# KlrShaK/opencv-SimpleSLAM

Measured on AMD Instinct MI355X. Metric: frames/sec ALIKED+LightGlue @1241x376, higher is better.
Workload: dtype f32 (contractions: f16 hi/lo split operands, f32 accumulate; 3 MFMA per product, 2 in attention's P.V = precision 'f16x3p1', the default since r05: profiles/r05_flip_soak.md, r06_flip_soak.md); 1 GPU; C2/C4: synthetic 1241x376x3 uint8 frame stream, ALIKED-n16 extract + LightGlue match (t-1,t), 2048 kpts/frame, min_conf 0.7, random-init weights; inputs resident in HBM before the timed region, features and matches left on the device (the `pcie` leg times the same pipeline with per-round H2D of the frames and D2H of {count, pairs}); max_kpts=2048, lightglue_layers_executed=9, pairs_per_lightglue_launch=8, frames_per_aliked_launch=8

## Files before the change

### opencv-simpleslam_amd/csrc/al_plan.hpp

```cpp
#pragma once
#include <algorithm>
#include <cstddef>
#include <cstdio>

namespace sslam {

constexpr int AL_LONG_SIDE = 1024;
constexpr int AL_PAD_DIV = 32;
constexpr int MAX_FRAMES = 16;
constexpr int B1_SW = 30;
constexpr int B2_SW = 30;
constexpr int DCN3_CS = 1;
constexpr int DCN4_CS = 4;
constexpr int AGG_PRE = 13;
constexpr int ST_W = 32, ST_H = 8;
constexpr int PRE_LDS_MAX = 48 * 1024;
constexpr int NHALO = 10;
constexpr int NW_R = 48, NW_OW = 64 - 2 * NHALO, NW_OH = NW_R - 2 * NHALO;
constexpr int HBINS = 4096;
constexpr int COLLECT_PPT = 16;
constexpr int SEL_CAP = 8192;
constexpr int EDGE_CAP = 2048;
constexpr int CAND_CAP = 1024 * 1024;
constexpr int REFINE_KPB = 32;
constexpr int SDDH_KSPLIT = 4;

constexpr int al_cdiv(int a, int b) { return (a + b - 1) / b; }

struct Dims {
// ... 14 lines not shown
    int b1_strips, b1_nblk, b1_hs, b1_nb;
    int b2_strips, b2_nblk, b2_hs, b2_nb, b2_waves, b2_gx;
    int H2, W2, HW2, H3, W3, HW3, H4, W4, HW4;
    int pool3_gx, pool4_gx;
    int off3_gx, dcn3_gx, off4_gx, dcn4_gx;
    float mo3, mo4, mo;
    int gate2_gx, gate3_gx, gate4_gx, gate34_gx;
    float sy2, sx2, sy8, sx8, sy32, sx32;
    int agg_pre_gx;
    int tail_gx, tail_gy;
    int nbx, nby, n_tiles, nms_gx;
    int npx, collect_gx;
    ALAggTile agg_tile;
    float scale_x, scale_y;
    int pre_tw, pre_th, pre_gx, pre_gy, pre_cols, pre_rows, pre_raw, pre_lds;
};

inline ALPlan al_plan(int H, int W, int C, int F) {
    ALPlan p{};
    p.F = F; p.KF = SDDH_KSPLIT * F;
    Dims& d = p.d;
    d.H = H; d.W = W; d.C = C;
    const double ar = (double)W / (double)H;
    if (ar > 1.0) { d.h = (int)(AL_LONG_SIDE / ar); d.w = AL_LONG_SIDE; }
    else { d.h = AL_LONG_SIDE; d.w = (int)(AL_LONG_SIDE * ar); }
    const double fy = (double)H / d.h, fx = (double)W / d.w;
    p.blur = (fy > fx ? fy : fx) > 1.0;
    const double sgy = (fy - 1.0) / 2.0 > 0.001 ? (fy - 1.0) / 2.0 : 0.001, sgx = (fx - 1.0) / 2.0 > 0.001 ? (fx - 1.0) / 2.0 : 0.001;
    p.sy = (float)sgy; p.sx = (float)sgx;
    const double ksy = 2.0 * 2 * sgy, ksx = 2.0 * 2 * sgx;
// ... 18 lines not shown
    p.b2_waves = p.b2_strips * p.b2_nb * F;
    p.b2_gx = al_cdiv(p.b2_waves, 4);
    p.H3 = Hp / 8; p.W3 = Wp / 8; p.HW3 = p.H3 * p.W3;
    p.H4 = Hp / 32; p.W4 = Wp / 32; p.HW4 = p.H4 * p.W4;
    p.pool3_gx = al_cdiv(32 * p.HW3, 256); p.pool4_gx = al_cdiv(64 * p.HW4, 256);
    p.off3_gx = al_cdiv(p.W3, 32); p.dcn3_gx = DCN3_CS * al_cdiv(p.W3, 32);
    p.off4_gx = al_cdiv(p.W4, 32); p.dcn4_gx = DCN4_CS * al_cdiv(p.W4, 32);
    p.mo3 = (float)(p.H3 > p.W3 ? p.H3 : p.W3) / 4.0f;
    p.mo4 = (float)(p.H4 > p.W4 ? p.H4 : p.W4) / 4.0f;
    p.gate2_gx = al_cdiv(p.HW2, 256); p.gate3_gx = al_cdiv(32 * p.HW3, 256); p.gate4_gx = al_cdiv(32 * p.HW4, 256);
    p.gate34_gx = p.gate3_gx + p.gate4_gx;
    auto step = [](int full, int S) { return (float)(full / S - 1) / (float)(full - 1); };
    p.sy2 = step(Hp, 2); p.sx2 = step(Wp, 2); p.sy8 = step(Hp, 8); p.sx8 = step(Wp, 8);
    p.sy32 = step(Hp, 32); p.sx32 = step(Wp, 32);
    p.agg_pre_gx = al_cdiv(p.HW2 + p.HW3 + p.HW4, 256);
    p.tail_gx = al_cdiv(Wp, ST_W); p.tail_gy = al_cdiv(Hp, ST_H);
    p.nbx = al_cdiv(d.w, NW_OW); p.nby = al_cdiv(d.h, NW_OH); p.n_tiles = p.nbx * p.nby;
    p.nms_gx = al_cdiv(p.n_tiles, 4);
    p.npx = d.h * d.w;
    p.collect_gx = al_cdiv(p.npx, 256 * COLLECT_PPT);
    p.mo = (float)(d.h > d.w ? d.h : d.w) / 4.0f;
    p.agg_tile = F >= 4 ? ALAggTile::T64x128 : ALAggTile::T64x64;
    p.scale_x = (float)d.w / (float)W; p.scale_y = (float)d.h / (float)H;
    {
        static constexpr int ladder[][2] = {{64, 8}, {32, 8}, {32, 4}, {16, 4}, {16, 2}, {8, 2}, {8, 1}, {4, 1}};
        const int rx = p.blur ? p.kx / 2 : 0, ry = p.blur ? p.ky / 2 : 0, planes = C == 1 ? 1 : 3;
        for (const auto& t : ladder) {
            p.pre_tw = t[0]; p.pre_th = t[1];
            p.pre_cols = (int)(fx * (t[0] - 1)) + 4;
            p.pre_rows = (int)(fy * (t[1] - 1)) + 4 + 2 * ry;
// ... 84 lines not shown
```

### opencv-simpleslam_amd/csrc/aliked_kernels.hip

```cpp
#include "common.hpp"
#include "al_plan.hpp"
#include "gemm_f32.hpp"
#include <type_traits>
#include "gemm_f16x3.hpp"

namespace {

using sslam::f32x16;
using sslam::acc_row;
using sslam::GemmSmem;
using sslam::GemmA;
using sslam::gemm_mainloop;
using sslam::Dims;
using sslam::MAX_FRAMES; using sslam::B1_SW; using sslam::B2_SW; using sslam::DCN3_CS; using sslam::DCN4_CS; using sslam::AGG_PRE;
using sslam::ST_W; using sslam::ST_H; using sslam::NHALO; using sslam::NW_R; using sslam::NW_OW; using sslam::NW_OH; using sslam::HBINS;
using sslam::COLLECT_PPT; using sslam::SEL_CAP; using sslam::EDGE_CAP; using sslam::REFINE_KPB; using sslam::SDDH_KSPLIT;

constexpr float SELU_SCALE = 1.0507009873554804934193349852946f;
constexpr float SELU_ALPHA = 1.6732632423543772848170429916717f;
__device__ __forceinline__ float selu(float x) {
    return SELU_SCALE * (x > 0.0f ? x : SELU_ALPHA * (__expf(x) - 1.0f));
}

__device__ __forceinline__ float selu_precise(float x) {
// ... 772 lines not shown
        for (int j = 0; j < MT * 4; ++j) {
            const int qi = wave * MT * 4 + j, m = qi / 16, r = qi % 16, co = 32 * (mt0 + m) + acc_row(r, lane);
            const int o = (m * 16 + r) * 64 + lane;
            float v = ((red[o] + red[o + MT * 1024]) + red[o + 2 * MT * 1024]) + red[o + 3 * MT * 1024];
            v += beta[co];
            if (RC) v += bd[co];
            v = selu(v);
            out[(size_t)co * HW + pix] = v;
            if (out_cl) out_cl[(size_t)pix * COUT + co] = v;
        }
    }
}



template <int CIN>
__global__ __launch_bounds__(256) void al_gate_kernel(const float* __restrict__ in, float* __restrict__ out,
                                                      int HW, const float* __restrict__ w ,
                                                      float* __restrict__ out_cl , size_t fs) {
    __shared__ float cl[256 * 33];
    const int p0 = blockIdx.x * blockDim.x, p = p0 + threadIdx.x, pc = min(p, HW - 1);
    in = fsh(in, blockIdx.y, fs); out = fsh(out, blockIdx.y, fs); out_cl = fsh(out_cl, blockIdx.y, fs);
    float v[CIN];
#pragma unroll
    for (int ci = 0; ci < CIN; ++ci) v[ci] = in[(size_t)ci * HW + pc];
    float acc[32];
#pragma unroll
    for (int o = 0; o < 32; ++o) acc[o] = 0.0f;
#pragma unroll
    for (int ci = 0; ci < CIN; ++ci) {
        const float* wp = w + ci * 32;
#pragma unroll
        for (int o = 0; o < 32; ++o) acc[o] = fmaf(v[ci], wp[o], acc[o]);
    }
#pragma unroll
    for (int o = 0; o < 32; ++o) { acc[o] = selu(acc[o]); cl[threadIdx.x * 33 + o] = acc[o]; }
    if (p < HW) {
#pragma unroll
        for (int o = 0; o < 32; ++o) out[(size_t)o * HW + p] = acc[o];
    }
    __syncthreads();
    const int npx = min(256, HW - p0);
    float* dst = out_cl + (size_t)p0 * 32;
    for (int i = threadIdx.x; i < npx * 8; i += 256) {
        const int q = i >> 3, c4 = (i & 7) * 4;
        *reinterpret_cast<float4*>(dst + (size_t)q * 32 + c4) = make_float4(cl[q * 33 + c4], cl[q * 33 + c4 + 1], cl[q * 33 + c4 + 2], cl[q * 33 + c4 + 3]);
    }
}

struct GateSmall { const float* in; float* out; int CIN; int HW; const float* w; float* out_cl; };
__global__ void al_gate_small_kernel(GateSmall a, GateSmall b, int blocks_a, size_t fs) {
    const bool second = (int)blockIdx.x >= blocks_a;
    const GateSmall& q = second ? b : a;
    const int i = ((int)blockIdx.x - (second ? blocks_a : 0)) * blockDim.x + threadIdx.x;
    const int CIN = q.CIN, HW = q.HW;
    if (i >= 32 * HW) return;
    const float* __restrict__ in = fsh(q.in, blockIdx.y, fs);
    float* __restrict__ out = fsh(q.out, blockIdx.y, fs);
    float* __restrict__ out_cl = fsh0(q.out_cl, blockIdx.y, fs);
    const float* __restrict__ w = q.w;
    const int co = i / HW, p = i % HW;
    float a0 = 0.0f, a1 = 0.0f;
#pragma unroll 8
    for (int ci = 0; ci < CIN; ci += 2) {
        a0 = fmaf(in[(size_t)ci * HW + p], w[ci * 32 + co], a0);
        a1 = fmaf(in[(size_t)(ci + 1) * HW + p], w[(ci + 1) * 32 + co], a1);
    }
    const float v = selu(a0 + a1);
    out[i] = v;
    out_cl[(size_t)p * 32 + co] = v;
}

struct Pyr {
    const float* x1; const float* g2; const float* g3; const float* g4;
    const float* w1;
    int Hp, Wp;
    float* g1cl;
    float sy2, sx2, sy8, sx8, sy32, sx32;
    const float *g2cl, *g3cl, *g4cl;
    const float *pre2, *pre3, *pre4;
};

__device__ __forceinline__ Pyr pyr_at(Pyr P, int f, size_t fs) {
    P.x1 = fsh(P.x1, f, fs); P.g2 = fsh(P.g2, f, fs); P.g3 = fsh(P.g3, f, fs); P.g4 = fsh(P.g4, f, fs);
    P.g1cl = fsh(P.g1cl, f, fs); P.g2cl = fsh(P.g2cl, f, fs); P.g3cl = fsh(P.g3cl, f, fs); P.g4cl = fsh(P.g4cl, f, fs);
    P.pre2 = fsh(P.pre2, f, fs); P.pre3 = fsh(P.pre3, f, fs); P.pre4 = fsh(P.pre4, f, fs);
    return P;
}

struct UpTap { int o00, o01, o10, o11; float w00, w01, w10, w11; };

__device__ __forceinline__ UpTap up_tap(int y, int x, int Hp, int Wp, int S, float sy, float sx) {
    const int ih = Hp / S, iw = Wp / S;
    const float fy = sy * (float)y, fx = sx * (float)x;
    const int y0 = (int)fy, x0 = (int)fx;
    const int y1 = y0 + (y0 < ih - 1), x1 = x0 + (x0 < iw - 1);
    const float ly = fy - (float)y0, lx = fx - (float)x0, hy = 1.0f - ly, hx = 1.0f - lx;
    UpTap t;
    t.o00 = y0 * iw + x0; t.o01 = y0 * iw + x1; t.o10 = y1 * iw + x0; t.o11 = y1 * iw + x1;
    t.w00 = hx; t.w01 = lx; t.w10 = hy; t.w11 = ly;
    return t;
}
__device__ __forceinline__ float up_eval_cl(const float* __restrict__ p, const UpTap& t, int c) {
    return t.w10 * (t.w00 * p[t.o00 * 32 + c] + t.w01 * p[t.o01 * 32 + c]) +
           t.w11 * (t.w00 * p[t.o10 * 32 + c] + t.w01 * p[t.o11 * 32 + c]);
}
__device__ __forceinline__ float up_eval(const float* __restrict__ p, const UpTap& t) {
    return t.w10 * (t.w00 * p[t.o00] + t.w01 * p[t.o01]) + t.w11 * (t.w00 * p[t.o10] + t.w01 * p[t.o11]);
}

constexpr int PRE_UNROLL = 32;
__global__ __launch_bounds__(256) void al_agg_pre_kernel(const float* __restrict__ g2cl , const float* __restrict__ g3cl,
                                                         const float* __restrict__ g4cl, const float* __restrict__ ws0 ,
                                                         float* __restrict__ pre2, float* __restrict__ pre3, float* __restrict__ pre4,
                                                         int Hp, int Wp, size_t fs) {
    const int f = blockIdx.y;
    const int n2 = (Hp / 2) * (Wp / 2), n3 = (Hp / 8) * (Wp / 8), n4 = (Hp / 32) * (Wp / 32);
    int i = blockIdx.x * blockDim.x + threadIdx.x;
    const float* g; float* pre; int S, lvl;
    if (i < n2) { g = g2cl; pre = pre2; S = 2; lvl = 1; }
    else if (i < n2 + n3) { i -= n2; g = g3cl; pre = pre3; S = 8; lvl = 2; }
    else if (i < n2 + n3 + n4) { i -= n2 + n3; g = g4cl; pre = pre4; S = 32; lvl = 3; }
    else return;
    g = fsh(g, f, fs); pre = fsh(pre, f, fs);
    const int ih = Hp / S, iw = Wp / S, n = ih * iw;
    const int y = i / iw, x = i % iw;
    const int xr = x + (x < iw - 1), yd = y + (y < ih - 1);
    const int ia = y * iw + x, ib = y * iw + xr, ic = yd * iw + x, id = yd * iw + xr;
    float pr[8] = {}, ss = 0.0f, hh = 0.0f, vv = 0.0f, d1 = 0.0f, d2 = 0.0f;
    const float* w = ws0 + lvl * 32 * 8;
#pragma unroll PRE_UNROLL
    for (int c = 0; c < 32; ++c) {
        const float* gc = g + (size_t)c * n;
        const float av = gc[ia], bv = gc[ib], cv = gc[ic], dv = gc[id];
        ss = fmaf(av, av, ss); hh = fmaf(av, bv, hh); vv = fmaf(av, cv, vv);
        d1 = fmaf(av, dv, d1); d2 = fmaf(bv, cv, d2);
#pragma unroll
        for (int o = 0; o < 8; ++o) pr[o] = fmaf(av, w[c * 8 + o], pr[o]);
    }
#pragma unroll
    for (int o = 0; o < 8; ++o) pre[(size_t)o * n + i] = pr[o];
    pre[(size_t)8 * n + i] = ss; pre[(size_t)9 * n + i] = hh; pre[(size_t)10 * n + i] = vv;
    pre[(size_t)11 * n + i] = d1; pre[(size_t)12 * n + i] = d2;
}

__device__ __forceinline__ void agg_level(const float* __restrict__ pre, int n, const UpTap& t, float (&s)[8], float& n2) {
#pragma unroll
    for (int o = 0; o < 8; ++o) s[o] += up_eval(pre + (size_t)o * n, t);
    const float w00 = t.w10 * t.w00, w01 = t.w10 * t.w01, w10 = t.w11 * t.w00, w11 = t.w11 * t.w01;
    const float* S = pre + (size_t)8 * n; const float* H = pre + (size_t)9 * n; const float* V = pre + (size_t)10 * n;
    const float* D1 = pre + (size_t)11 * n; const float* D2 = pre + (size_t)12 * n;
    const float sq = (w00 * w00 * S[t.o00] + w01 * w01 * S[t.o01]) + (w10 * w10 * S[t.o10] + w11 * w11 * S[t.o11]);
    const float cr = ((w00 * w01) * H[t.o00] + (w10 * w11) * H[t.o10]) + ((w00 * w10) * V[t.o00] + (w01 * w11) * V[t.o01]) +
                     ((w00 * w11) * D1[t.o00] + (w01 * w10) * D2[t.o00]);
    n2 += fmaf(2.0f, cr, sq);
}

constexpr int AGG1_UNROLL = 2;
// ... 5 lines not shown
    __shared__ float g1s[256 * 33];
    const int x = blockIdx.x * blockDim.x + threadIdx.x, y = blockIdx.y;
    const bool live = x < P.Wp;
    const size_t HW = (size_t)P.Hp * P.Wp, pix = (size_t)y * P.Wp + min(x, P.Wp - 1);
    float xv[16];
#pragma unroll
    for (int k = 0; k < 16; ++k) xv[k] = P.x1[k * HW + pix];
    float s[8];
#pragma unroll
    for (int o = 0; o < 8; ++o) s[o] = 0.0f;
    float n2 = 0.0f;
#pragma unroll AGG1_UNROLL
    for (int c = 0; c < 32; ++c) {
        float a = 0.0f;
#pragma unroll
        for (int k = 0; k < 16; ++k) a = fmaf(xv[k], P.w1[k * 32 + c], a);
        a = selu_precise(a);
        g1s[threadIdx.x * 33 + c] = a;
        n2 = fmaf(a, a, n2);
#pragma unroll
        for (int o = 0; o < 8; ++o) s[o] = fmaf(a, ws0[c * 8 + o], s[o]);
    }
    const UpTap t2 = up_tap(y, x, P.Hp, P.Wp, 2, P.sy2, P.sx2), t3 = up_tap(y, x, P.Hp, P.Wp, 8, P.sy8, P.sx8),
                t4 = up_tap(y, x, P.Hp, P.Wp, 32, P.sy32, P.sx32);
    agg_level(P.pre2, (int)(HW / 4), t2, s, n2);
    agg_level(P.pre3, (int)(HW / 64), t3, s, n2);
    agg_level(P.pre4, (int)(HW / 1024), t4, s, n2);
    if (live) {
#pragma unroll
        for (int o = 0; o < 8; ++o) s8[o * HW + pix] = selu_precise(s[o]);
        rnorm[pix] = 1.0f / fmaxf(sqrtf(n2), 1e-12f);
    }
    __builtin_amdgcn_fence(__ATOMIC_RELEASE, "workgroup");
    __builtin_amdgcn_s_barrier();
    __builtin_amdgcn_fence(__ATOMIC_ACQUIRE, "workgroup");
    typedef float f32x4_t __attribute__((ext_vector_type(4)));
    const int npx = min(256, P.Wp - (int)(blockIdx.x * blockDim.x));
    float* dst = P.g1cl + ((size_t)y * P.Wp + blockIdx.x * blockDim.x) * 32;
    for (int i = threadIdx.x; i < npx * 8; i += 256) {
        const int p = i >> 3, c4 = (i & 7) * 4;
        const f32x4_t v = {g1s[p * 33 + c4], g1s[p * 33 + c4 + 1], g1s[p * 33 + c4 + 2], g1s[p * 33 + c4 + 3]};
        *reinterpret_cast<f32x4_t*>(dst + (size_t)p * 32 + c4) = v;
    }
}

__device__ __forceinline__ float2 feat_pair(const Pyr& P, const float* __restrict__ rnorm, int pl, int pt,
                                            int y, int x, int lane) {
    const int yp = y + pt, xp = x + pl;
    const size_t pix = (size_t)yp * P.Wp + xp;
    float a, b;
    const int c = lane & 31;
    if (lane < 32) {
        a = P.g1cl[pix * 32 + c];
        b = up_eval_cl(P.g3cl, up_tap(yp, xp, P.Hp, P.Wp, 8, P.sy8, P.sx8), c);
    } else {
        a = up_eval_cl(P.g2cl, up_tap(yp, xp, P.Hp, P.Wp, 2, P.sy2, P.sx2), c);
        b = up_eval_cl(P.g4cl, up_tap(yp, xp, P.Hp, P.Wp, 32, P.sy32, P.sx32), c);
// ... 757 lines not shown
struct sslam_aliked {
    sslam_ctx* ctx = nullptr;
    int max_h = 0, max_w = 0, max_kpts = 0;
    int max_frames = 1;
    size_t fs = 0;
    int Hp_cap = 0, Wp_cap = 0;
    sslam::OwnedSlab slab;
    float* blob = nullptr;
    ALConvW b1c1, b1c2, b2c1, b2c2;
    const float *b2dw, *b2db;
    ALDcnW b3c1, b3c2, b4c1, b4c2;
    const float *b3dw, *b3db, *b4dw, *b4db;
    _Float16 *b3c1of, *b3c2of, *b4c1of, *b4c2of;
    _Float16 *b3c1f, *b3c2f, *b4c1f, *b4c2f;
    const float *gw1, *gw2, *gw3, *gw4;
    const float *sh0, *sh2, *sh4, *sh6;
    const float *d_ow, *d_ob, *d_w2, *d_b2, *d_sf, *d_agg;
    ALCtrl* ctrl;
    uint8_t* in_u8;
    float *img, *x1, *x2, *p3, *off, *t3, *x3, *p4, *t4, *x4, *g2, *g3, *g4;
    float *s8, *rnorm, *score, *nms, *bsum, *gk, *g1cl, *g2cl, *g3cl, *g4cl, *pre2, *pre3, *pre4;
    unsigned long long* cand;
    unsigned* hist;
    int cand_cap;
    int* kp_index;
    int* range_sticky;
    unsigned long long* sel_keys;
    float *kp_norm, *kp_score, *patch, *h32, *pos, *sampled, *feats, *raw;
    _Float16 *d_sf_s, *d_agg_s;
    _Float16* b2c2f;
// ... 39 lines not shown
    (void)hipGetLastError();
    const Dims& d = p.d;
    const sslam::ALKptPlan& k = g->kp;
    const int F = p.F, KF = p.KF, NK = k.NK;
    const size_t fs = g->fs;
    const dim3 b256(256);
    hipLaunchKernelGGL(al_reset_kernel, dim3(F), b256, 0, s, g->ctrl, g->hist, fs, g->gk, p.kx, p.sx, p.ky, p.sy);

    hipLaunchKernelGGL(al_preprocess_kernel, dim3(p.pre_gx, p.pre_gy, F), b256, (size_t)p.pre_lds, s, srcs, g->img, d, g->gk, p.kx, p.ky,
                       p.blur, PreTile{p.pre_tw, p.pre_th, p.pre_cols, p.pre_rows, p.pre_raw}, fs);
    hipLaunchKernelGGL(al_block1_rows_kernel, dim3(p.b1_strips, p.b1_nb, F), dim3(64), 0, s, g->img, g->x1, d.Hp, d.Wp, p.b1_hs,
                       g->b1c1.w, g->b1c1.a, g->b1c1.b, g->b1c2f, g->b1c2.a, g->b1c2.b, g->ctrl, fs);
    hipLaunchKernelGGL(al_block2_rows_kernel, dim3(p.b2_gx), b256, B2_LDS, s, g->x1, g->x2, p.H2, p.W2, p.b2_hs, p.b2_nb, p.b2_strips,
                       p.b2_waves, g->b2c1f, g->b2c2f, g->b2c1.a, g->b2c1.b, g->b2db, g->b2c2.a, g->b2c2.b, g->ctrl, fs);
    const dim3 off3 = dim3(p.off3_gx, p.H3, F), dcn3 = dim3(p.dcn3_gx, p.H3, F);
    hipLaunchKernelGGL(al_avgpool_kernel, dim3(p.pool3_gx, F), b256, 0, s, g->x2, g->p3, 32, p.H2, p.W2, 4, fs, g->p3cl);
    hipLaunchKernelGGL((al_offset_conv_h_kernel<32>), off3, b256, 0, s, g->p3cl, g->off, p.H3, p.W3, g->b3c1of, g->b3c1.ob, p.mo3, g->ctrl, fs);
    hipLaunchKernelGGL((al_dcn_h_kernel<32, 64, 0, DCN3_CS>), dcn3, b256, 0, s, g->p3cl, g->off, nullptr, p.H3, p.W3, g->b3c1f, g->b3c1.b, nullptr, g->t3, g->t3cl, g->ctrl, fs);
    hipLaunchKernelGGL((al_offset_conv_h_kernel<64>), off3, b256, 0, s, g->t3cl, g->off, p.H3, p.W3, g->b3c2of, g->b3c2.ob, p.mo3, g->ctrl, fs);
    hipLaunchKernelGGL((al_dcn_h_kernel<64, 64, 32, DCN3_CS>), dcn3, b256, 0, s, g->t3cl, g->off, g->p3cl, p.H3, p.W3, g->b3c2f, g->b3c2.b, g->b3db, g->x3, nullptr, g->ctrl, fs);
    const dim3 off4 = dim3(p.off4_gx, p.H4, F), dcn4 = dim3(p.dcn4_gx, p.H4, F);
    sslam::graph_cut(s);
    hipLaunchKernelGGL(al_avgpool_kernel, dim3(p.pool4_gx, F), b256, 0, s, g->x3, g->p4, 64, p.H3, p.W3, 4, fs, g->p4cl);
    hipLaunchKernelGGL((al_offset_conv_h_kernel<64>), off4, b256, 0, s, g->p4cl, g->off, p.H4, p.W4, g->b4c1of, g->b4c1.ob, p.mo4, g->ctrl, fs);
    hipLaunchKernelGGL((al_dcn_h_kernel<64, 128, 0, DCN4_CS>), dcn4, b256, 0, s, g->p4cl, g->off, nullptr, p.H4, p.W4, g->b4c1f, g->b4c1.b, nullptr, g->t4, g->t4cl, g->ctrl, fs);
    hipLaunchKernelGGL((al_offset_conv_h_kernel<128>), off4, b256, 0, s, g->t4cl, g->off, p.H4, p.W4, g->b4c2of, g->b4c2.ob, p.mo4, g->ctrl, fs);
    hipLaunchKernelGGL((al_dcn_h_kernel<128, 128, 64, DCN4_CS>), dcn4, b256, 0, s, g->t4cl, g->off, g->p4cl, p.H4, p.W4, g->b4c2f, g->b4c2.b, g->b4db, g->x4, nullptr, g->ctrl, fs);
    hipLaunchKernelGGL(al_gate_kernel<32>, dim3(p.gate2_gx, F), b256, 0, s, g->x2, g->g2, p.HW2, g->gw2, g->g2cl, fs);
    hipLaunchKernelGGL(al_gate_small_kernel, dim3(p.gate34_gx, F), b256, 0, s, GateSmall{g->x3, g->g3, 64, p.HW3, g->gw3, g->g3cl},
                       GateSmall{g->x4, g->g4, 128, p.HW4, g->gw4, g->g4cl}, p.gate3_gx, fs);
    Pyr P{g->x1, g->g2, g->g3, g->g4, g->gw1, d.Hp, d.Wp, g->g1cl};
    P.sy2 = p.sy2; P.sx2 = p.sx2; P.sy8 = p.sy8; P.sx8 = p.sx8; P.sy32 = p.sy32; P.sx32 = p.sx32;
    P.g2cl = g->g2cl; P.g3cl = g->g3cl; P.g4cl = g->g4cl;
    P.pre2 = g->pre2; P.pre3 = g->pre3; P.pre4 = g->pre4;
    hipLaunchKernelGGL(al_agg_pre_kernel, dim3(p.agg_pre_gx, F), b256, 0, s, g->g2, g->g3, g->g4, g->sh0, g->pre2, g->pre3, g->pre4,
                       d.Hp, d.Wp, fs);
    hipLaunchKernelGGL(al_aggregate_kernel, dim3(p.pad_gx, d.Hp, F), b256, 0, s, P, g->sh0, g->s8, g->rnorm, fs);
    hipLaunchKernelGGL(al_score_tail_kernel, dim3(p.tail_gx, p.tail_gy, F), dim3(ST_T), 0, s, g->s8, d.Hp, d.Wp, g->sh2, g->sh4, g->sh6,
                       g->score, d.h, d.w, d.pl, d.pt, fs);
    hipLaunchKernelGGL(al_nms_wave_kernel, dim3(p.nms_gx, F), b256, 0, s, g->score, d.h, d.w, p.nbx, p.n_tiles, g->nms, g->bsum, 0.2f,
                       g->cand, g->cand_cap, g->ctrl, g->hist, fs);
    sslam::graph_cut(s);
    hipLaunchKernelGGL(al_collect_kernel, dim3(p.collect_gx, F), b256, 0, s, g->nms, p.npx, 0.0f, 1, g->bsum, p.n_tiles, g->cand,
                       g->cand_cap, g->ctrl, g->hist, fs);
    hipLaunchKernelGGL(al_select_kernel, dim3(F), dim3(1024), SEL_LDS, s, g->cand, g->cand_cap, n_limit, g->sel_keys, g->ctrl, g->hist, fs);
    hipLaunchKernelGGL(al_refine_kernel, dim3(k.refine_gx, F), b256, 0, s, g->score, d.h, d.w, g->sel_keys, g->kp_index, g->kp_norm,
                       g->kp_score, g->ctrl, fs);
    hipLaunchKernelGGL(al_patch_kernel, dim3(k.patch_gx, F), b256, 0, s, P, g->rnorm, d.pl, d.pt, d.h, d.w, g->kp_norm, g->patch, g->ctrl, fs);
    hipLaunchKernelGGL((al_gemm_kernel<64, 64, 1, 1>), dim3(1, k.rows64, KF), b256, 0, s, g->patch, 1152, g->d_ow, nullptr, 32, g->h32,
                       1, NK, 0, g->ctrl, SDDH_KSPLIT, fs);
    hipLaunchKernelGGL(al_offsets_kernel, dim3(k.offsets_gx, F), b256, 0, s, g->h32, NK, g->d_ob, g->d_w2, g->d_b2, g->kp_norm, d.h, d.w,
// ... 48 lines not shown
    g->ctx = ctx; g->max_h = max_h; g->max_w = max_w; g->max_kpts = max_kpts; g->max_frames = max_frames;
    g->kp = sslam::al_kpt_plan(max_kpts);
    g->Hp_cap = sslam::AL_LONG_SIDE + sslam::AL_PAD_DIV; g->Wp_cap = sslam::AL_LONG_SIDE + sslam::AL_PAD_DIV;
    const sslam::ALExtents e = sslam::al_extents((size_t)g->Hp_cap * g->Wp_cap, (size_t)max_h * max_w, (size_t)max_kpts);
    g->cand_cap = sslam::CAND_CAP;
    auto bind_shared = [&](sslam::Slab& A) {
        g->blob = A.take<float>(n_floats);
        g->d_sf_s = A.take<_Float16>(2 * 128 * 128); g->d_agg_s = A.take<_Float16>((size_t)2 * 128 * 2048);
        g->b2c2f = A.take<_Float16>(2 * 32 * 288);
        g->b1c2f = A.take<_Float16>(5 * 2 * 64 * 8);
        g->b2c1f = A.take<_Float16>(10 * 2 * 64 * 8);
        g->b3c1f = A.take<_Float16>((size_t)(9 * 2 + 0) * 2 * 2 * 512); g->b3c2f = A.take<_Float16>((size_t)(9 * 4 + 2) * 2 * 2 * 512);
        g->b4c1f = A.take<_Float16>((size_t)(9 * 4 + 0) * 4 * 2 * 512); g->b4c2f = A.take<_Float16>((size_t)(9 * 8 + 4) * 4 * 2 * 512);
        g->b3c1of = A.take<_Float16>(18 * 2 * 512); g->b3c2of = A.take<_Float16>(36 * 2 * 512); g->b4c1of = A.take<_Float16>(36 * 2 * 512); g->b4c2of = A.take<_Float16>(72 * 2 * 512);
        g->gk = A.take<float>(64);
        g->range_sticky = A.take<int>(4);
    };
    auto bind_frame = [&](sslam::Slab& A) {
        g->ctrl = A.take<ALCtrl>(e.ctrl);
        g->in_u8 = A.take<uint8_t>(e.in_u8);
        g->img = A.take<float>(e.img);
        g->x1 = A.take<float>(e.x1); g->x2 = A.take<float>(e.x2);
        g->p3 = A.take<float>(e.p3); g->off = A.take<float>(e.off);
        g->t3 = A.take<float>(e.t3); g->x3 = A.take<float>(e.x3);
        g->p3cl = A.take<float>(e.p3cl); g->t3cl = A.take<float>(e.t3cl);
        g->p4cl = A.take<float>(e.p4cl); g->t4cl = A.take<float>(e.t4cl);
        g->p4 = A.take<float>(e.p4); g->t4 = A.take<float>(e.t4); g->x4 = A.take<float>(e.x4);
        g->g2 = A.take<float>(e.g2); g->g3 = A.take<float>(e.g3); g->g4 = A.take<float>(e.g4);
        g->g2cl = A.take<float>(e.g2cl); g->g3cl = A.take<float>(e.g3cl); g->g4cl = A.take<float>(e.g4cl);
        g->s8 = A.take<float>(e.s8); g->rnorm = A.take<float>(e.rnorm); g->g1cl = A.take<float>(e.g1cl);
// ... 26 lines not shown
        hipStream_t s = ctx->stream;
        SSLAM_HIP_CHECK(hipMemsetAsync(g->range_sticky, 0, 4 * sizeof(int), s));
        hipLaunchKernelGGL(al_conv32_wfrag_kernel, dim3(sslam::cdiv(32 * 288, 256)), dim3(256), 0, s, g->b2c2.w, g->b2c2f, g->range_sticky);
        hipLaunchKernelGGL(al_conv16_wfrag_kernel, dim3(sslam::cdiv(5 * 64 * 8, 256)), dim3(256), 0, s, g->b1c2.w, g->b1c2f, g->range_sticky);
        hipLaunchKernelGGL(al_conv32p_wfrag_kernel, dim3(sslam::cdiv(10 * 64 * 8, 256)), dim3(256), 0, s, g->b2c1.w, g->b2dw, g->b2c1f, g->range_sticky);
        hipLaunchKernelGGL(al_split_kernel, dim3(sslam::cdiv(128 * 128, 256)), dim3(256), 0, s, g->d_sf, g->d_sf_s, (size_t)128 * 128, g->range_sticky);
        hipLaunchKernelGGL(al_split_kernel, dim3(sslam::cdiv(128 * 2048, 256)), dim3(256), 0, s, g->d_agg, g->d_agg_s, (size_t)128 * 2048, g->range_sticky);
        hipLaunchKernelGGL((al_dcn_wfrag_kernel<32, 64, 0>), dim3(sslam::cdiv((9 * 2 + 0) * 2 * 512, 256)), dim3(256), 0, s, g->b3c1.w, g->b3c1.a, nullptr, g->b3c1f, g->range_sticky);
        hipLaunchKernelGGL((al_dcn_wfrag_kernel<64, 64, 32>), dim3(sslam::cdiv((9 * 4 + 2) * 2 * 512, 256)), dim3(256), 0, s, g->b3c2.w, g->b3c2.a, g->b3dw, g->b3c2f, g->range_sticky);
        hipLaunchKernelGGL((al_dcn_wfrag_kernel<64, 128, 0>), dim3(sslam::cdiv((9 * 4 + 0) * 4 * 512, 256)), dim3(256), 0, s, g->b4c1.w, g->b4c1.a, nullptr, g->b4c1f, g->range_sticky);
        hipLaunchKernelGGL((al_dcn_wfrag_kernel<128, 128, 64>), dim3(sslam::cdiv((9 * 8 + 4) * 4 * 512, 256)), dim3(256), 0, s, g->b4c2.w, g->b4c2.a, g->b4dw, g->b4c2f, g->range_sticky);
        hipLaunchKernelGGL(al_offc_wfrag_kernel<32>, dim3(sslam::cdiv(18 * 512, 256)), dim3(256), 0, s, g->b3c1.ow, g->b3c1of, g->range_sticky);
        hipLaunchKernelGGL(al_offc_wfrag_kernel<64>, dim3(sslam::cdiv(36 * 512, 256)), dim3(256), 0, s, g->b3c2.ow, g->b3c2of, g->range_sticky);
        hipLaunchKernelGGL(al_offc_wfrag_kernel<64>, dim3(sslam::cdiv(36 * 512, 256)), dim3(256), 0, s, g->b4c1.ow, g->b4c1of, g->range_sticky);
        hipLaunchKernelGGL(al_offc_wfrag_kernel<128>, dim3(sslam::cdiv(72 * 512, 256)), dim3(256), 0, s, g->b4c2.ow, g->b4c2of, g->range_sticky);
        int wflag = 0;
        SSLAM_HIP_CHECK(hipMemcpyAsync(&wflag, g->range_sticky, sizeof(int), hipMemcpyDeviceToHost, s));
        SSLAM_HIP_CHECK(hipStreamSynchronize(s));
        SSLAM_REQUIRE(!wflag, "sslam_aliked_create: a weight (BN scale folded) with |value| >= 65520 does not fit the fp16 planes "
                              "of the split-precision stages");
    }
    SSLAM_HIP_CHECK(hipFuncSetAttribute((const void*)al_block2_rows_kernel, hipFuncAttributeMaxDynamicSharedMemorySize, (int)B2_LDS));
    SSLAM_HIP_CHECK(hipFuncSetAttribute((const void*)al_select_kernel, hipFuncAttributeMaxDynamicSharedMemorySize, SEL_LDS));
    sslam::ctx_retain(ctx);
    *out = g.release();
    return 0;
}

int sslam_aliked_create(sslam_ctx* ctx, const float* weights, size_t n_floats, int max_h, int max_w,
                        int max_kpts, sslam_aliked** out) {
// ... 117 lines not shown
            dims[0] = d.h; dims[1] = d.w; dims[2] = d.Hp; dims[3] = d.Wp; dims[4] = d.pl; dims[5] = d.pt;
            dims[6] = c.n_cand; dims[7] = c.n_kp;
            SSLAM_REQUIRE(bytes <= sizeof(dims), "sslam_aliked_debug_read: dims is 32 bytes");
            memcpy(dst, dims, bytes);
            return 0;
        }
        case 3: src = g->x1; cap = e.x1 * 4; break;
        case 4: src = g->x2; cap = e.x2 * 4; break;
        case 5: src = g->x3; cap = e.x3 * 4; break;
        case 6: src = g->x4; cap = e.x4 * 4; break;
        case 7: src = g->img; cap = e.img * 4; break;
        case 8: src = g->nms; cap = (size_t)d.h * d.w * 4; break;
        case 9: src = g->kp_norm; cap = (size_t)g->max_kpts * 8; break;
        case 10: src = g->g1cl; cap = e.g1cl * 4; break;
        case 11: src = g->rnorm; cap = e.rnorm * 4; break;
        case 12: src = g->g2; cap = e.g2 * 4; break;
        case 13: src = g->g3; cap = e.g3 * 4; break;
        case 14: src = g->g4; cap = e.g4 * 4; break;
        case 15: src = g->pre2; cap = e.pre2 * 4; break;
        case 16: src = g->pre3; cap = e.pre3 * 4; break;
        case 17: src = g->pre4; cap = e.pre4 * 4; break;
        case 18: src = g->s8; cap = e.s8 * 4; break;
        case 19: src = g->pos; cap = (size_t)g->max_kpts * 32 * 4; break;
        case 20: src = g->patch; cap = (size_t)g->max_kpts * 1152 * 4; break;
        default: SSLAM_REQUIRE(false, "sslam_aliked_debug_read: unknown buffer %d", which);
    }
    SSLAM_REQUIRE(bytes <= cap, "sslam_aliked_debug_read: %zu bytes requested, buffer has %zu", bytes, cap);
    SSLAM_HIP_CHECK(hipMemcpy(dst, src, bytes, hipMemcpyDeviceToHost));
    return 0;
}

}
```

Baseline: 1267 frames/s.

## Fuse ALIKED level gates, avgpool and aggregation pre-planes into per-level tiled kernels

Replaces the separate avgpool, gate and agg_pre kernels with a tiled level-2 kernel and a combined level-3/4 kernel. Each one computes the SELU gate into LDS with a one-pixel halo, produces the channel-last gate output and the 13 pre-planes from LDS, and for level 2 also computes the 4x4 average pool. The planar g2/g3/g4 writes are removed, and debug reads now rebuild them on demand. It also transposes w1 once at creation for contiguous weight access, and moves the upsample aggregation after the g1 store in the aggregate kernel. The aim is fewer launches and less HBM traffic, at the cost of redundant halo gate computation and higher LDS use.

```diff
diff --git a/opencv-simpleslam_amd/csrc/al_plan.hpp b/opencv-simpleslam_amd/csrc/al_plan.hpp
--- a/opencv-simpleslam_amd/csrc/al_plan.hpp
+++ b/opencv-simpleslam_amd/csrc/al_plan.hpp
@@ -13,6 +13,8 @@
 constexpr int DCN3_CS = 1;
 constexpr int DCN4_CS = 4;
 constexpr int AGG_PRE = 13;
+constexpr int L2_TW = 32, L2_TH = 8;
+constexpr int LS_TW = 16, LS_TH = 4;
 constexpr int ST_W = 32, ST_H = 8;
 constexpr int PRE_LDS_MAX = 48 * 1024;
 constexpr int NHALO = 10;
@@ -57,6 +59,8 @@
     ALAggTile agg_tile;
     float scale_x, scale_y;
     int pre_tw, pre_th, pre_gx, pre_gy, pre_cols, pre_rows, pre_raw, pre_lds;
+    int lvl2_gx, lvl2_gy;
+    int lvl3_gx, lvl3_n, lvl4_gx, lvl4_n, lvl34_n;
 };
 
 inline ALPlan al_plan(int H, int W, int C, int F) {
@@ -105,6 +109,10 @@
     p.sy2 = step(Hp, 2); p.sx2 = step(Wp, 2); p.sy8 = step(Hp, 8); p.sx8 = step(Wp, 8);
     p.sy32 = step(Hp, 32); p.sx32 = step(Wp, 32);
     p.agg_pre_gx = al_cdiv(p.HW2 + p.HW3 + p.HW4, 256);
+    p.lvl2_gx = al_cdiv(p.W2, L2_TW); p.lvl2_gy = al_cdiv(p.H2, L2_TH);
+    p.lvl3_gx = al_cdiv(p.W3, LS_TW); p.lvl3_n = p.lvl3_gx * al_cdiv(p.H3, LS_TH);
+    p.lvl4_gx = al_cdiv(p.W4, LS_TW); p.lvl4_n = p.lvl4_gx * al_cdiv(p.H4, LS_TH);
+    p.lvl34_n = p.lvl3_n + p.lvl4_n;
     p.tail_gx = al_cdiv(Wp, ST_W); p.tail_gy = al_cdiv(Hp, ST_H);
     p.nbx = al_cdiv(d.w, NW_OW); p.nby = al_cdiv(d.h, NW_OH); p.n_tiles = p.nbx * p.nby;
     p.nms_gx = al_cdiv(p.n_tiles, 4);
diff --git a/opencv-simpleslam_amd/csrc/aliked_kernels.hip b/opencv-simpleslam_amd/csrc/aliked_kernels.hip
--- a/opencv-simpleslam_amd/csrc/aliked_kernels.hip
+++ b/opencv-simpleslam_amd/csrc/aliked_kernels.hip
@@ -810,66 +810,9 @@
 
 
 
-template <int CIN>
-__global__ __launch_bounds__(256) void al_gate_kernel(const float* __restrict__ in, float* __restrict__ out,
-                                                      int HW, const float* __restrict__ w ,
-                                                      float* __restrict__ out_cl , size_t fs) {
-    __shared__ float cl[256 * 33];
-    const int p0 = blockIdx.x * blockDim.x, p = p0 + threadIdx.x, pc = min(p, HW - 1);
-    in = fsh(in, blockIdx.y, fs); out = fsh(out, blockIdx.y, fs); out_cl = fsh(out_cl, blockIdx.y, fs);
-    float v[CIN];
-#pragma unroll
-    for (int ci = 0; ci < CIN; ++ci) v[ci] = in[(size_t)ci * HW + pc];
-    float acc[32];
-#pragma unroll
-    for (int o = 0; o < 32; ++o) acc[o] = 0.0f;
-#pragma unroll
-    for (int ci = 0; ci < CIN; ++ci) {
-        const float* wp = w + ci * 32;
-#pragma unroll
-        for (int o = 0; o < 32; ++o) acc[o] = fmaf(v[ci], wp[o], acc[o]);
-    }
-#pragma unroll
-    for (int o = 0; o < 32; ++o) { acc[o] = selu(acc[o]); cl[threadIdx.x * 33 + o] = acc[o]; }
-    if (p < HW) {
-#pragma unroll
-        for (int o = 0; o < 32; ++o) out[(size_t)o * HW + p] = acc[o];
-    }
-    __syncthreads();
-    const int npx = min(256, HW - p0);
-    float* dst = out_cl + (size_t)p0 * 32;
-    for (int i = threadIdx.x; i < npx * 8; i += 256) {
-        const int q = i >> 3, c4 = (i & 7) * 4;
-        *reinterpret_cast<float4*>(dst + (size_t)q * 32 + c4) = make_float4(cl[q * 33 + c4], cl[q * 33 + c4 + 1], cl[q * 33 + c4 + 2], cl[q * 33 + c4 + 3]);
-    }
-}
-
-struct GateSmall { const float* in; float* out; int CIN; int HW; const float* w; float* out_cl; };
-__global__ void al_gate_small_kernel(GateSmall a, GateSmall b, int blocks_a, size_t fs) {
-    const bool second = (int)blockIdx.x >= blocks_a;
-    const GateSmall& q = second ? b : a;
-    const int i = ((int)blockIdx.x - (second ? blocks_a : 0)) * blockDim.x + threadIdx.x;
-    const int CIN = q.CIN, HW = q.HW;
-    if (i >= 32 * HW) return;
-    const float* __restrict__ in = fsh(q.in, blockIdx.y, fs);
-    float* __restrict__ out = fsh(q.out, blockIdx.y, fs);
-    float* __restrict__ out_cl = fsh0(q.out_cl, blockIdx.y, fs);
-    const float* __restrict__ w = q.w;
-    const int co = i / HW, p = i % HW;
-    float a0 = 0.0f, a1 = 0.0f;
-#pragma unroll 8
-    for (int ci = 0; ci < CIN; ci += 2) {
-        a0 = fmaf(in[(size_t)ci * HW + p], w[ci * 32 + co], a0);
-        a1 = fmaf(in[(size_t)(ci + 1) * HW + p], w[(ci + 1) * 32 + co], a1);
-    }
-    const float v = selu(a0 + a1);
-    out[i] = v;
-    out_cl[(size_t)p * 32 + co] = v;
-}
-
 struct Pyr {
-    const float* x1; const float* g2; const float* g3; const float* g4;
-    const float* w1;
+    const float* x1;
+    const float* w1t;
     int Hp, Wp;
     float* g1cl;
     float sy2, sx2, sy8, sx8, sy32, sx32;
@@ -878,7 +821,7 @@
 };
 
 __device__ __forceinline__ Pyr pyr_at(Pyr P, int f, size_t fs) {
-    P.x1 = fsh(P.x1, f, fs); P.g2 = fsh(P.g2, f, fs); P.g3 = fsh(P.g3, f, fs); P.g4 = fsh(P.g4, f, fs);
+    P.x1 = fsh(P.x1, f, fs);
     P.g1cl = fsh(P.g1cl, f, fs); P.g2cl = fsh(P.g2cl, f, fs); P.g3cl = fsh(P.g3cl, f, fs); P.g4cl = fsh(P.g4cl, f, fs);
     P.pre2 = fsh(P.pre2, f, fs); P.pre3 = fsh(P.pre3, f, fs); P.pre4 = fsh(P.pre4, f, fs);
     return P;
@@ -905,30 +848,13 @@
     return t.w10 * (t.w00 * p[t.o00] + t.w01 * p[t.o01]) + t.w11 * (t.w00 * p[t.o10] + t.w01 * p[t.o11]);
 }
 
-constexpr int PRE_UNROLL = 32;
-__global__ __launch_bounds__(256) void al_agg_pre_kernel(const float* __restrict__ g2cl , const float* __restrict__ g3cl,
-                                                         const float* __restrict__ g4cl, const float* __restrict__ ws0 ,
-                                                         float* __restrict__ pre2, float* __restrict__ pre3, float* __restrict__ pre4,
-                                                         int Hp, int Wp, size_t fs) {
-    const int f = blockIdx.y;
-    const int n2 = (Hp / 2) * (Wp / 2), n3 = (Hp / 8) * (Wp / 8), n4 = (Hp / 32) * (Wp / 32);
-    int i = blockIdx.x * blockDim.x + threadIdx.x;
-    const float* g; float* pre; int S, lvl;
-    if (i < n2) { g = g2cl; pre = pre2; S = 2; lvl = 1; }
-    else if (i < n2 + n3) { i -= n2; g = g3cl; pre = pre3; S = 8; lvl = 2; }
-    else if (i < n2 + n3 + n4) { i -= n2 + n3; g = g4cl; pre = pre4; S = 32; lvl = 3; }
-    else return;
-    g = fsh(g, f, fs); pre = fsh(pre, f, fs);
-    const int ih = Hp / S, iw = Wp / S, n = ih * iw;
-    const int y = i / iw, x = i % iw;
-    const int xr = x + (x < iw - 1), yd = y + (y < ih - 1);
-    const int ia = y * iw + x, ib = y * iw + xr, ic = yd * iw + x, id = yd * iw + xr;
+__device__ __forceinline__ void pre_planes_lds(const float* __restrict__ cl, int ia, int row, const float* __restrict__ w ,
+                                               float* __restrict__ pre, int n, int i) {
+    const int ib = ia + 33, ic = ia + row * 33, id = ic + 33;
     float pr[8] = {}, ss = 0.0f, hh = 0.0f, vv = 0.0f, d1 = 0.0f, d2 = 0.0f;
-    const float* w = ws0 + lvl * 32 * 8;
-#pragma unroll PRE_UNROLL
+#pragma unroll
     for (int c = 0; c < 32; ++c) {
-        const float* gc = g + (size_t)c * n;
-        const float av = gc[ia], bv = gc[ib], cv = gc[ic], dv = gc[id];
+        const float av = cl[ia + c], bv = cl[ib + c], cv = cl[ic + c], dv = cl[id + c];
         ss = fmaf(av, av, ss); hh = fmaf(av, bv, hh); vv = fmaf(av, cv, vv);
         d1 = fmaf(av, dv, d1); d2 = fmaf(bv, cv, d2);
 #pragma unroll
@@ -938,6 +864,138 @@
     for (int o = 0; o < 8; ++o) pre[(size_t)o * n + i] = pr[o];
     pre[(size_t)8 * n + i] = ss; pre[(size_t)9 * n + i] = hh; pre[(size_t)10 * n + i] = vv;
     pre[(size_t)11 * n + i] = d1; pre[(size_t)12 * n + i] = d2;
+}
+
+__device__ __forceinline__ void gate32_px(const float* __restrict__ in, int HW, int pc, const float* __restrict__ w, float (&v)[32], float (&acc)[32]) {
+#pragma unroll
+    for (int ci = 0; ci < 32; ++ci) v[ci] = in[(size_t)ci * HW + pc];
+#pragma unroll
+    for (int o = 0; o < 32; ++o) acc[o] = 0.0f;
+#pragma unroll
+    for (int ci = 0; ci < 32; ++ci) {
+        const float* wp = w + ci * 32;
+#pragma unroll
+        for (int o = 0; o < 32; ++o) acc[o] = fmaf(v[ci], wp[o], acc[o]);
+    }
+#pragma unroll
+    for (int o = 0; o < 32; ++o) acc[o] = selu(acc[o]);
+}
+
+constexpr int L2_PW = sslam::L2_TW + 1, L2_NP = L2_PW * (sslam::L2_TH + 1), L2_HALO = sslam::L2_TW + sslam::L2_TH + 1;
+static_assert(sslam::L2_TW == 32 && sslam::L2_TH == 8 && sslam::L2_TW * sslam::L2_TH == 256 && L2_HALO <= 64, "a thread per interior pixel, tile rows of 32 lanes, the halo in wave 0");
+__global__ __launch_bounds__(256) void al_level2_kernel(const float* __restrict__ x2 , int H, int W, const float* __restrict__ w ,
+                                                        const float* __restrict__ ws0l , float* __restrict__ gcl ,
+                                                        float* __restrict__ pre , float* __restrict__ p3 ,
+                                                        float* __restrict__ p3cl , size_t fs) {
+    __shared__ float cl[L2_NP * 33];
+    const Tile3 b = xcd_band();
+    x2 = fsh(x2, b.z, fs); gcl = fsh(gcl, b.z, fs); pre = fsh(pre, b.z, fs); p3 = fsh(p3, b.z, fs); p3cl = fsh(p3cl, b.z, fs);
+    const int HW = H * W, x0 = b.x * sslam::L2_TW, y0 = b.y * sslam::L2_TH;
+    const int tx = threadIdx.x & 31, ty = threadIdx.x >> 5, x = x0 + tx, y = y0 + ty;
+    const int lp = (ty * L2_PW + tx) * 33;
+    float v[32], acc[32];
+    gate32_px(x2, HW, min(y, H - 1) * W + min(x, W - 1), w, v, acc);
+#pragma unroll
+    for (int ci = 0; ci < 32; ++ci) cl[lp + ci] = v[ci];
+    __syncthreads();
+    {
+        const int c = threadIdx.x & 31, H3 = H / 4, W3 = W / 4;
+        for (int k = threadIdx.x >> 5; k < 16; k += 8) {
+            const int bx = k & 7, by = k >> 3, X3 = x0 / 4 + bx, Y3 = y0 / 4 + by;
+            if (X3 >= W3 || Y3 >= H3) continue;
+            float u[16];
+#pragma unroll
+            for (int a = 0; a < 4; ++a)
+#pragma unroll
+                for (int e = 0; e < 4; ++e) u[4 * a + e] = cl[((by * 4 + a) * L2_PW + bx * 4 + e) * 33 + c];
+            float s = 0.0f;
+#pragma unroll
+            for (int q = 0; q < 16; ++q) s += u[q];
+            const float m = s / 16.0f;
+            p3[(size_t)c * (H3 * W3) + Y3 * W3 + X3] = m;
+            p3cl[(size_t)(Y3 * W3 + X3) * 32 + c] = m;
+        }
+    }
+    __syncthreads();
+#pragma unroll
+    for (int o = 0; o < 32; ++o) cl[lp + o] = acc[o];
+    if (threadIdx.x < L2_HALO) {
+        const int h = threadIdx.x;
+        const int hr = h < sslam::L2_TH ? h : sslam::L2_TH, hc = h < sslam::L2_TH ? sslam::L2_TW : (h - sslam::L2_TH);
+        gate32_px(x2, HW, min(y0 + hr, H - 1) * W + min(x0 + hc, W - 1), w, v, acc);
+        const int hp = (hr * L2_PW + hc) * 33;
+#pragma unroll
+        for (int o = 0; o < 32; ++o) cl[hp + o] = acc[o];
+    }
+    __syncthreads();
+    for (int i = threadIdx.x; i < 256 * 8; i += 256) {
+        const int q = i >> 3, c4 = (i & 7) * 4, r = q >> 5, cc = q & 31;
+        if (x0 + cc < W && y0 + r < H) {
+            const float* s = cl + (r * L2_PW + cc) * 33 + c4;
+            *reinterpret_cast<float4*>(gcl + ((size_t)(y0 + r) * W + x0 + cc) * 32 + c4) = make_float4(s[0], s[1], s[2], s[3]);
+        }
+    }
+    if (x < W && y < H) pre_planes_lds(cl, lp, L2_PW, ws0l, pre, HW, y * W + x);
+}
+
+constexpr int LS_PW = sslam::LS_TW + 1, LS_NP = LS_PW * (sslam::LS_TH + 1);
+constexpr int LS_SMEM = LS_NP * (128 + 4) + LS_NP * 33;
+static_assert(sslam::LS_TW * sslam::LS_TH <= 256 && LS_SMEM * 4 <= 64 * 1024, "a thread per interior pixel for the planes; static LDS");
+struct LevelSmall { const float* in; int H, W; const float* w; const float* ws0l; float* gcl; float* pre; int gx; };
+template <int CIN>
+__device__ __forceinline__ void level_small_tile(const LevelSmall& q, int tile, int f, size_t fs, float* __restrict__ smem) {
+    constexpr int XS = CIN + 4;
+    float* xs = smem;
+    float* gs = smem + LS_NP * XS;
+    const float* __restrict__ in = fsh(q.in, f, fs);
+    float* __restrict__ gcl = fsh(q.gcl, f, fs);
+    float* __restrict__ pre = fsh(q.pre, f, fs);
+    const int H = q.H, W = q.W, HW = H * W;
+    const int x0 = (tile % q.gx) * sslam::LS_TW, y0 = (tile / q.gx) * sslam::LS_TH;
+    for (int e = threadIdx.x; e < CIN * LS_NP; e += 256) {
+        const int ci = e / LS_NP, pp = e - ci * LS_NP, r = pp / LS_PW, c = pp - r * LS_PW;
+        xs[pp * XS + ci] = in[(size_t)ci * HW + min(y0 + r, H - 1) * W + min(x0 + c, W - 1)];
+    }
+    const int co = threadIdx.x & 31;
+    float wr[CIN];
+#pragma unroll
+    for (int ci = 0; ci < CIN; ++ci) wr[ci] = q.w[ci * 32 + co];
+    __syncthreads();
+#pragma unroll 1
+    for (int pp = threadIdx.x >> 5; pp < LS_NP; pp += 8) {
+        const float4* xp = reinterpret_cast<const float4*>(xs + pp * XS);
+        float a0 = 0.0f, a1 = 0.0f;
+#pragma unroll
+        for (int k = 0; k < CIN / 4; ++k) {
+            const float4 t = xp[k];
+            a0 = fmaf(t.x, wr[4 * k], a0); a1 = fmaf(t.y, wr[4 * k + 1], a1);
+            a0 = fmaf(t.z, wr[4 * k + 2], a0); a1 = fmaf(t.w, wr[4 * k + 3], a1);
+        }
+        const float g = selu(a0 + a1);
+        gs[pp * 33 + co] = g;
+        const int r = pp / LS_PW, c = pp - r * LS_PW;
+        if (r < sslam::LS_TH && c < sslam::LS_TW && y0 + r < H && x0 + c < W) gcl[((size_t)(y0 + r) * W + x0 + c) * 32 + co] = g;
+    }
+    __syncthreads();
+    if (threadIdx.x < sslam::LS_TW * sslam::LS_TH) {
+        const int tx = threadIdx.x % sslam::LS_TW, ty = threadIdx.x / sslam::LS_TW, x = x0 + tx, y = y0 + ty;
+        if (x < W && y < H) pre_planes_lds(gs, (ty * LS_PW + tx) * 33, LS_PW, q.ws0l, pre, HW, y * W + x);
+    }
+}
+__global__ __launch_bounds__(256) void al_level_small_kernel(LevelSmall a, LevelSmall b, int blocks_a, size_t fs) {
+    __shared__ __attribute__((aligned(16))) float smem[LS_SMEM];
+    if ((int)blockIdx.x < blocks_a) level_small_tile<64>(a, (int)blockIdx.x, (int)blockIdx.y, fs, smem);
+    else level_small_tile<128>(b, (int)blockIdx.x - blocks_a, (int)blockIdx.y, fs, smem);
+}
+
+__global__ void al_w1t_kernel(const float* __restrict__ w1, float* __restrict__ w1t) {
+    const int i = blockIdx.x * blockDim.x + threadIdx.x;
+    if (i < 16 * 32) w1t[(i % 32) * 16 + i / 32] = w1[i];
+}
+
+__global__ void al_cl_to_planar_kernel(const float* __restrict__ cl, float* __restrict__ planar, int n) {
+    const int i = blockIdx.x * blockDim.x + threadIdx.x;
+    if (i < 32 * n) planar[i] = cl[(size_t)(i % n) * 32 + i / n];
 }
 
 __device__ __forceinline__ void agg_level(const float* __restrict__ pre, int n, const UpTap& t, float (&s)[8], float& n2) {
@@ -973,22 +1031,12 @@
     for (int c = 0; c < 32; ++c) {
         float a = 0.0f;
 #pragma unroll
-        for (int k = 0; k < 16; ++k) a = fmaf(xv[k], P.w1[k * 32 + c], a);
+        for (int k = 0; k < 16; ++k) a = fmaf(xv[k], P.w1t[c * 16 + k], a);
         a = selu_precise(a);
         g1s[threadIdx.x * 33 + c] = a;
         n2 = fmaf(a, a, n2);
 #pragma unroll
         for (int o = 0; o < 8; ++o) s[o] = fmaf(a, ws0[c * 8 + o], s[o]);
-    }
-    const UpTap t2 = up_tap(y, x, P.Hp, P.Wp, 2, P.sy2, P.sx2), t3 = up_tap(y, x, P.Hp, P.Wp, 8, P.sy8, P.sx8),
-                t4 = up_tap(y, x, P.Hp, P.Wp, 32, P.sy32, P.sx32);
-    agg_level(P.pre2, (int)(HW / 4), t2, s, n2);
-    agg_level(P.pre3, (int)(HW / 64), t3, s, n2);
-    agg_level(P.pre4, (int)(HW / 1024), t4, s, n2);
-    if (live) {
-#pragma unroll
-        for (int o = 0; o < 8; ++o) s8[o * HW + pix] = selu_precise(s[o]);
-        rnorm[pix] = 1.0f / fmaxf(sqrtf(n2), 1e-12f);
     }
     __builtin_amdgcn_fence(__ATOMIC_RELEASE, "workgroup");
     __builtin_amdgcn_s_barrier();
@@ -1000,6 +1048,16 @@
         const int p = i >> 3, c4 = (i & 7) * 4;
         const f32x4_t v = {g1s[p * 33 + c4], g1s[p * 33 + c4 + 1], g1s[p * 33 + c4 + 2], g1s[p * 33 + c4 + 3]};
         *reinterpret_cast<f32x4_t*>(dst + (size_t)p * 32 + c4) = v;
+    }
+    const UpTap t2 = up_tap(y, x, P.Hp, P.Wp, 2, P.sy2, P.sx2), t3 = up_tap(y, x, P.Hp, P.Wp, 8, P.sy8, P.sx8),
+                t4 = up_tap(y, x, P.Hp, P.Wp, 32, P.sy32, P.sx32);
+    agg_level(P.pre2, (int)(HW / 4), t2, s, n2);
+    agg_level(P.pre3, (int)(HW / 64), t3, s, n2);
+    agg_level(P.pre4, (int)(HW / 1024), t4, s, n2);
+    if (live) {
+#pragma unroll
+        for (int o = 0; o < 8; ++o) s8[o * HW + pix] = selu_precise(s[o]);
+        rnorm[pix] = 1.0f / fmaxf(sqrtf(n2), 1e-12f);
     }
 }
 
@@ -1787,6 +1845,7 @@
     _Float16 *b3c1of, *b3c2of, *b4c1of, *b4c2of;
     _Float16 *b3c1f, *b3c2f, *b4c1f, *b4c2f;
     const float *gw1, *gw2, *gw3, *gw4;
+    float* gw1t;
     const float *sh0, *sh2, *sh4, *sh6;
     const float *d_ow, *d_ob, *d_w2, *d_b2, *d_sf, *d_agg;
     ALCtrl* ctrl;
@@ -1856,7 +1915,8 @@
     hipLaunchKernelGGL(al_block2_rows_kernel, dim3(p.b2_gx), b256, B2_LDS, s, g->x1, g->x2, p.H2, p.W2, p.b2_hs, p.b2_nb, p.b2_strips,
                        p.b2_waves, g->b2c1f, g->b2c2f, g->b2c1.a, g->b2c1.b, g->b2db, g->b2c2.a, g->b2c2.b, g->ctrl, fs);
     const dim3 off3 = dim3(p.off3_gx, p.H3, F), dcn3 = dim3(p.dcn3_gx, p.H3, F);
-    hipLaunchKernelGGL(al_avgpool_kernel, dim3(p.pool3_gx, F), b256, 0, s, g->x2, g->p3, 32, p.H2, p.W2, 4, fs, g->p3cl);
+    hipLaunchKernelGGL(al_level2_kernel, dim3(p.lvl2_gx, p.lvl2_gy, F), b256, 0, s, g->x2, p.H2, p.W2, g->gw2, g->sh0 + 1 * 32 * 8, g->g2cl,
+                       g->pre2, g->p3, g->p3cl, fs);
     hipLaunchKernelGGL((al_offset_conv_h_kernel<32>), off3, b256, 0, s, g->p3cl, g->off, p.H3, p.W3, g->b3c1of, g->b3c1.ob, p.mo3, g->ctrl, fs);
     hipLaunchKernelGGL((al_dcn_h_kernel<32, 64, 0, DCN3_CS>), dcn3, b256, 0, s, g->p3cl, g->off, nullptr, p.H3, p.W3, g->b3c1f, g->b3c1.b, nullptr, g->t3, g->t3cl, g->ctrl, fs);
     hipLaunchKernelGGL((al_offset_conv_h_kernel<64>), off3, b256, 0, s, g->t3cl, g->off, p.H3, p.W3, g->b3c2of, g->b3c2.ob, p.mo3, g->ctrl, fs);
@@ -1868,15 +1928,13 @@
     hipLaunchKernelGGL((al_dcn_h_kernel<64, 128, 0, DCN4_CS>), dcn4, b256, 0, s, g->p4cl, g->off, nullptr, p.H4, p.W4, g->b4c1f, g->b4c1.b, nullptr, g->t4, g->t4cl, g->ctrl, fs);
     hipLaunchKernelGGL((al_offset_conv_h_kernel<128>), off4, b256, 0, s, g->t4cl, g->off, p.H4, p.W4, g->b4c2of, g->b4c2.ob, p.mo4, g->ctrl, fs);
     hipLaunchKernelGGL((al_dcn_h_kernel<128, 128, 64, DCN4_CS>), dcn4, b256, 0, s, g->t4cl, g->off, g->p4cl, p.H4, p.W4, g->b4c2f, g->b4c2.b, g->b4db, g->x4, nullptr, g->ctrl, fs);
-    hipLaunchKernelGGL(al_gate_kernel<32>, dim3(p.gate2_gx, F), b256, 0, s, g->x2, g->g2, p.HW2, g->gw2, g->g2cl, fs);
-    hipLaunchKernelGGL(al_gate_small_kernel, dim3(p.gate34_gx, F), b256, 0, s, GateSmall{g->x3, g->g3, 64, p.HW3, g->gw3, g->g3cl},
-                       GateSmall{g->x4, g->g4, 128, p.HW4, g->gw4, g->g4cl}, p.gate3_gx, fs);
-    Pyr P{g->x1, g->g2, g->g3, g->g4, g->gw1, d.Hp, d.Wp, g->g1cl};
+    hipLaunchKernelGGL(al_level_small_kernel, dim3(p.lvl34_n, F), b256, 0, s,
+                       LevelSmall{g->x3, p.H3, p.W3, g->gw3, g->sh0 + 2 * 32 * 8, g->g3cl, g->pre3, p.lvl3_gx},
+                       LevelSmall{g->x4, p.H4, p.W4, g->gw4, g->sh0 + 3 * 32 * 8, g->g4cl, g->pre4, p.lvl4_gx}, p.lvl3_n, fs);
+    Pyr P{g->x1, g->gw1t, d.Hp, d.Wp, g->g1cl};
     P.sy2 = p.sy2; P.sx2 = p.sx2; P.sy8 = p.sy8; P.sx8 = p.sx8; P.sy32 = p.sy32; P.sx32 = p.sx32;
     P.g2cl = g->g2cl; P.g3cl = g->g3cl; P.g4cl = g->g4cl;
     P.pre2 = g->pre2; P.pre3 = g->pre3; P.pre4 = g->pre4;
-    hipLaunchKernelGGL(al_agg_pre_kernel, dim3(p.agg_pre_gx, F), b256, 0, s, g->g2, g->g3, g->g4, g->sh0, g->pre2, g->pre3, g->pre4,
-                       d.Hp, d.Wp, fs);
     hipLaunchKernelGGL(al_aggregate_kernel, dim3(p.pad_gx, d.Hp, F), b256, 0, s, P, g->sh0, g->s8, g->rnorm, fs);
     hipLaunchKernelGGL(al_score_tail_kernel, dim3(p.tail_gx, p.tail_gy, F), dim3(ST_T), 0, s, g->s8, d.Hp, d.Wp, g->sh2, g->sh4, g->sh6,
                        g->score, d.h, d.w, d.pl, d.pt, fs);
@@ -1955,6 +2013,7 @@
         g->b4c1f = A.take<_Float16>((size_t)(9 * 4 + 0) * 4 * 2 * 512); g->b4c2f = A.take<_Float16>((size_t)(9 * 8 + 4) * 4 * 2 * 512);
         g->b3c1of = A.take<_Float16>(18 * 2 * 512); g->b3c2of = A.take<_Float16>(36 * 2 * 512); g->b4c1of = A.take<_Float16>(36 * 2 * 512); g->b4c2of = A.take<_Float16>(72 * 2 * 512);
         g->gk = A.take<float>(64);
+        g->gw1t = A.take<float>(32 * 16);
         g->range_sticky = A.take<int>(4);
     };
     auto bind_frame = [&](sslam::Slab& A) {
@@ -2011,6 +2070,7 @@
         hipLaunchKernelGGL(al_offc_wfrag_kernel<64>, dim3(sslam::cdiv(36 * 512, 256)), dim3(256), 0, s, g->b3c2.ow, g->b3c2of, g->range_sticky);
         hipLaunchKernelGGL(al_offc_wfrag_kernel<64>, dim3(sslam::cdiv(36 * 512, 256)), dim3(256), 0, s, g->b4c1.ow, g->b4c1of, g->range_sticky);
         hipLaunchKernelGGL(al_offc_wfrag_kernel<128>, dim3(sslam::cdiv(72 * 512, 256)), dim3(256), 0, s, g->b4c2.ow, g->b4c2of, g->range_sticky);
+        hipLaunchKernelGGL(al_w1t_kernel, dim3(2), dim3(256), 0, s, g->gw1, g->gw1t);
         int wflag = 0;
         SSLAM_HIP_CHECK(hipMemcpyAsync(&wflag, g->range_sticky, sizeof(int), hipMemcpyDeviceToHost, s));
         SSLAM_HIP_CHECK(hipStreamSynchronize(s));
@@ -2158,9 +2218,18 @@
         case 9: src = g->kp_norm; cap = (size_t)g->max_kpts * 8; break;
         case 10: src = g->g1cl; cap = e.g1cl * 4; break;
         case 11: src = g->rnorm; cap = e.rnorm * 4; break;
-        case 12: src = g->g2; cap = e.g2 * 4; break;
-        case 13: src = g->g3; cap = e.g3 * 4; break;
-        case 14: src = g->g4; cap = e.g4 * 4; break;
+        case 12: case 13: case 14: {
+            const int lv = which - 12, S = lv == 0 ? 2 : lv == 1 ? 8 : 32, n = (d.Hp / S) * (d.Wp / S);
+            const float* cl = lv == 0 ? g->g2cl : lv == 1 ? g->g3cl : g->g4cl;
+            float* planar = lv == 0 ? g->g2 : lv == 1 ? g->g3 : g->g4;
+            cap = (lv == 0 ? e.g2 : lv == 1 ? e.g3 : e.g4) * 4;
+            SSLAM_REQUIRE(n > 0 && d.Hp <= g->Hp_cap && d.Wp <= g->Wp_cap, "sslam_aliked_debug_read: no admitted frame to read level %d of", lv + 2);
+            hipLaunchKernelGGL(al_cl_to_planar_kernel, dim3(sslam::cdiv(32 * n, 256)), dim3(256), 0, g->ctx->stream, cl, planar, n);
+            SSLAM_HIP_CHECK(hipGetLastError());
+            SSLAM_HIP_CHECK(hipStreamSynchronize(g->ctx->stream));
+            src = planar;
+            break;
+        }
         case 15: src = g->pre2; cap = e.pre2 * 4; break;
         case 16: src = g->pre3; cap = e.pre3 * 4; break;
         case 17: src = g->pre4; cap = e.pre4 * 4; break;
```

Result: faster. 1281 frames/s (median of 6 runs) (+1.1%).
